# aleksandrina-streltsova/lidar-global-registration

Measured on AMD Instinct MI355X. Metric: scan-pair registrations/sec, higher is better.
Workload: dtype f32

## Files before the change

lidar-global-registration_amd/csrc/lgr_align.hip:

```cpp
#include <rocprim/device/device_scan.hpp>

#include <chrono>
#include <cmath>

#include <climits>

#include "lgr_internal.h"

namespace {

__device__ __forceinline__ float corr_threshold(float a, float b, float dthr) {
    float m = (a < b) ? b : a;
    return (dthr < m) ? dthr : m;
}

template <int KMAX>
__device__ __forceinline__ float cluster_distance(int i, int j, int k, const int32_t* __restrict__ knn_a, const int32_t* __restrict__ knn_b,
                                                   const int32_t* __restrict__ ab_idx) {
    int nb[KMAX];
#pragma unroll
    for (int b = 0; b < KMAX; ++b) nb[b] = b < k ? knn_b[(size_t) j * k + b] : -2;
    int consistent = 0, pairs = 0;
    for (int a0 = 0; a0 < k; a0 += 8) {
        int in[8], mt[8];
// ... 105 lines not shown
    size_t tb = 0;
    LGR_HIP(ctx, rocprim::exclusive_scan(nullptr, tb, flags, pos, 0, (size_t) ns, rocprim::plus<int>(), ctx->stream));
    void* tmp;
    LGR_TRY(lgr_ws(ctx, WS_GRID_TMP, tb, &tmp));
    LGR_HIP(ctx, rocprim::exclusive_scan(tmp, tb, flags, pos, 0, (size_t) ns, rocprim::plus<int>(), ctx->stream));
    filter_emit<<<cdiv(ns, 256), 256, 0, ctx->stream>>>(ns, d_ij_idx, flags, pos, dist, thr_s, thr_t, distance_thr, d_out);
    int* h;
    LGR_TRY(lgr_pinned(ctx, 64, (void**) &h));
    LGR_HIP(ctx, hipMemcpyAsync(h, pos + (ns - 1), 4, hipMemcpyDeviceToHost, ctx->stream));
    LGR_HIP(ctx, hipMemcpyAsync(h + 1, flags + (ns - 1), 4, hipMemcpyDeviceToHost, ctx->stream));
    LGR_HIP(ctx, hipStreamSynchronize(ctx->stream));
    *n_out = h[0] + h[1];
    LGR_HIP(ctx, hipGetLastError());
    return LGR_OK;
}

static void tick(lgr_ctx* ctx, int i) { (void) hipEventRecord(ctx->ev[i], ctx->stream); }

__global__ void gather_rows12_kernel(const float* __restrict__ pts, const int32_t* __restrict__ idx, int m, float* __restrict__ out) {
    size_t e = (size_t) blockIdx.x * blockDim.x + threadIdx.x;
    if (e >= (size_t) m * 12) return;
    out[e] = pts[(size_t) idx[e / 12] * 12 + e % 12];
}
static void gather_rows12(lgr_ctx* ctx, const float* pts, const int32_t* idx, int m, float* out) {
    gather_rows12_kernel<<<cdiv((long long) m * 12, 256), 256, 0, ctx->stream>>>(pts, idx, m, out);
}
__global__ void finalize_kernel(lgr_corr* __restrict__ corr, int n, const int32_t* __restrict__ ks, const int32_t* __restrict__ kt) {
    int i = blockIdx.x * blockDim.x + threadIdx.x;
    if (i >= n) return;
    corr[i].index_query = ks[corr[i].index_query];
    corr[i].index_match = kt[corr[i].index_match];
}

typedef int (*FeatureStage)(lgr_ctx* ctx, const float* kps, int m, const float* surf, int n, float radius, float* out, const lgr_params* p, const float* vp);
struct Descriptor {
    int len;
    FeatureStage stage;
    bool dense;
    int lrf;
};
static int fpfh_stage(lgr_ctx* ctx, const float* kps, int m, const float* surf, int n, float radius, float* out, const lgr_params*, const float*) { return lgr_fpfh_dev(ctx, kps, m, surf, n, radius, out); }
static int shot_stage(lgr_ctx* ctx, const float* kps, int m, const float* surf, int n, float radius, float* out, const lgr_params*, const float*) { return lgr_shot_dev(ctx, kps, m, surf, n, radius, nullptr, out, nullptr); }
static int rops_stage(lgr_ctx* ctx, const float* kps, int m, const float* surf, int n, float radius, float* out, const lgr_params* p, const float* vp) {
    float* kn;
    LGR_TRY(lgr_ws_t(ctx, WS_ROPS_KPS, (size_t) m * 12, &kn));
    LGR_HIP(ctx, hipMemcpyAsync(kn, kps, (size_t) m * 48, hipMemcpyDeviceToDevice, ctx->stream));
    LGR_TRY(lgr_normals_knn_dev(ctx, kn, m, surf, n, p->normal_nr_points, vp, 1));
    return lgr_rops_gravity_dev(ctx, kn, m, surf, n, radius, out);
}
static const Descriptor DESCRIPTORS[] = {
     {33, fpfh_stage, false, LGR_LRF_DEFAULT},
     {352, shot_stage, true, LGR_LRF_DEFAULT},
     {135, rops_stage, true, LGR_LRF_GRAVITY},
};
static_assert(LGR_DESCRIPTOR_FPFH == 0 && LGR_DESCRIPTOR_SHOT == 1 && LGR_DESCRIPTOR_ROPS == 2, "DESCRIPTORS is indexed by descriptor_id");

extern "C" void lgr_default_feature_params(lgr_feature_params* f) {
    if (!f) return;
    memset(f, 0, sizeof(*f));
    f->descriptor_id = LGR_DESCRIPTOR_FPFH;
    f->lrf_id = LGR_LRF_DEFAULT;
}

static int feature_descriptor(lgr_ctx* ctx, const lgr_params* p, const lgr_feature_params* f, const Descriptor** out) {
    *out = &DESCRIPTORS[LGR_DESCRIPTOR_FPFH];
    if (!f) return LGR_OK;
    LGR_CHECK(ctx, f->descriptor_id >= 0 && f->descriptor_id < (int) (sizeof DESCRIPTORS / sizeof *DESCRIPTORS), LGR_ERR_UNSUPPORTED);
    const Descriptor& d = DESCRIPTORS[f->descriptor_id];
    if (d.dense) {
        LGR_CHECK(ctx, f->lrf_id == LGR_LRF_DEFAULT || f->lrf_id == LGR_LRF_GRAVITY || f->lrf_id == LGR_LRF_GT, LGR_ERR_INVALID_ARG);
        LGR_CHECK(ctx, f->lrf_id == d.lrf, LGR_ERR_UNSUPPORTED);
        LGR_CHECK(ctx, p->use_bfmatcher && !p->has_guess, LGR_ERR_UNSUPPORTED);
        LGR_CHECK(ctx, ctx->opt.arithmetic != LGR_ARITH_PCL, LGR_ERR_UNSUPPORTED);
    }
    *out = &d;
    return LGR_OK;
// ... 7 lines not shown
    int sizes[2], ksizes[2];
    int32_t* kidx[2] = {nullptr, nullptr};
    lgr_corr* d_out;
    int* n_out;
    bool empty = false;
    float *feat[2], *surf[2], *dij, *dji;
    int32_t *ij, *ji;
    FilterTables ftab;
    float ms[3] = {0, 0, 0};
    struct Tables {
        CorrCall* c;
        int operator()(lgr_ctx* cx) const {
            LGR_TRY(filter_cloud_tables(cx, c->kclouds[0], c->ksizes[0], c->p->cluster_k, c->ftab.thr_s, c->ftab.knn_s));
            return filter_cloud_tables(cx, c->kclouds[1], c->ksizes[1], c->p->cluster_k, c->ftab.thr_t, c->ftab.knn_t);
        }
    } tables{this};
    lgr_helper_guard tables_guard;
    struct PrepGuard { lgr_ctx* c; ~PrepGuard() { lgr_match_prepare_cancel(c); } } prep_guard;

    CorrCall(lgr_ctx* ctx, const float* d_src, int ns, const float* d_tgt, int nt, const lgr_params* p, lgr_corr* d_out, int* n_out)
        : ctx(ctx), p(p), clouds{d_src, d_tgt}, kclouds{d_src, d_tgt}, sizes{ns, nt}, ksizes{ns, nt}, d_out(d_out), n_out(n_out), prep_guard{ctx} {}
    CorrCall(const CorrCall&) = delete;
    const float* vp(int side) const { return side == 0 ? (p->has_vp_src ? p->vp_src : nullptr) : (p->has_vp_tgt ? p->vp_tgt : nullptr); }
    float iss_radius(int side) const { return side == 0 ? p->iss_radius_src : p->iss_radius_tgt; }
    bool both_dirs() const { return p->matching_id != LGR_MATCH_ONE_SIDED; }
};

static int level_features(lgr_ctx* cx, const CorrCall& c, int side, const float* in, int n_in, float voxel, float radius, float* surf,
                          const float* kps, int m, const int32_t* d_list, float* sub, float* out, float* ms, int* nd) {
    const lgr_params* p = c.p;
    tick(cx, 0);
    LGR_TRY(lgr_downsample_dev(cx, in, n_in, voxel, surf, nd));
    tick(cx, 1);
    LGR_TRY(lgr_normals_knn_dev(cx, surf, *nd, nullptr, 0, p->normal_nr_points, c.vp(side), p->normals_available));
    tick(cx, 2);
    if (m) {
        if (d_list) { gather_rows12(cx, kps, d_list, m, sub); kps = sub; }
        LGR_TRY(c.d->stage(cx, kps, m, surf, *nd, radius, out, p, c.vp(side)));
    }
    tick(cx, 3);
    LGR_HIP(cx, hipEventSynchronize(cx->ev[3]));
    float t;
    for (int s = 0; s < 3; ++s) { (void) hipEventElapsedTime(&t, cx->ev[s], cx->ev[s + 1]); ms[s] += t; }
    return LGR_OK;
}

struct MsSide {
    float iss_radius = 0.f;
    int min_l2 = INT_MAX, max_l2 = INT_MIN;
    std::vector<std::vector<int>> lists;
    std::vector<size_t> feat_off;
    float* feat = nullptr;
    int32_t* d_lists = nullptr;
    std::vector<float> xyz;
};

static int ms_initialize(CorrCall& c, int side, MsSide& st) {
    lgr_ctx* ctx = c.ctx;
    const lgr_params* p = c.p;
    const int D = c.d->len, n = c.sizes[side], n_kps = c.ksizes[side];
    const float *d_pcd = c.clouds[side], *d_kps = c.kclouds[side];
    st.iss_radius = c.iss_radius(side);
    const int k = 5;
    LGR_CHECK(ctx, n >= k, LGR_ERR_INVALID_ARG);
    int32_t* d_nn;
    float* d_d2;
    LGR_TRY(lgr_ws_t(ctx, WS_MS_KNN_I, (size_t) n_kps * k, &d_nn));
    LGR_TRY(lgr_ws_t(ctx, WS_MS_KNN_D, (size_t) n_kps * k, &d_d2));
    LGR_TRY(lgr_knn_dev(ctx, d_kps, n_kps, d_pcd, n, k, d_nn, d_d2));
    std::vector<float> d2((size_t) n_kps * k);
    std::vector<float> kp((size_t) n_kps * 12);
// ... 410 lines not shown
```

lidar-global-registration_amd/csrc/lgr_features.hip:

```cpp
#include <rocprim/device/device_radix_sort.hpp>
#include <rocprim/device/device_scan.hpp>

#include <algorithm>
#include <cmath>
#include <type_traits>
#include <unordered_map>
#include <vector>

#include "lgr_grid.cuh"
#include "lgr_knn_wave.cuh"
#include "lgr_seqsum.h"
#include "lgr_math.cuh"
#include "lgr_libm.cuh"

namespace {

__global__ void voxel_keys(const float* __restrict__ pts, int n, float bx, float by, float bz, float voxel,
                           unsigned long long* __restrict__ keys, int* __restrict__ vals, int* __restrict__ bad) {
    int i = blockIdx.x * blockDim.x + threadIdx.x;
    if (i >= n) return;
    float x = pts[(size_t) i * 12], y = pts[(size_t) i * 12 + 1], z = pts[(size_t) i * 12 + 2];
    unsigned long long k = ~0ull;
    if (lgr_finite3(x, y, z)) {
        int ix = (int) floorf((x - bx) / voxel), iy = (int) floorf((y - by) / voxel), iz = (int) floorf((z - bz) / voxel);
// ... 959 lines not shown
        out[i] = r;
    }
}
extern "C" int lgr_selfcheck_libm(lgr_ctx* ctx, int fn, const float* a, const float* b, long long n, float* out) {
    lgr_turn turn__(ctx);
    if (!ctx) return LGR_ERR_INVALID_ARG;
    LGR_CHECK(ctx, fn >= 0 && fn <= 6 && a && out && n >= 0 && (fn != 2 || b), LGR_ERR_INVALID_ARG);
    if (n == 0) return LGR_OK;
    LGR_HIP(ctx, hipSetDevice(ctx->device));
    float *da, *db, *dout;
    LGR_TRY(lgr_ws_t(ctx, WS_HOST_A, (size_t) n, &da));
    LGR_TRY(lgr_ws_t(ctx, WS_HOST_B, (size_t) n, &db));
    LGR_TRY(lgr_ws_t(ctx, WS_HOST_C, (size_t) n, &dout));
    LGR_HIP(ctx, hipMemcpyAsync(da, a, (size_t) n * 4, hipMemcpyHostToDevice, ctx->stream));
    if (fn == 2) LGR_HIP(ctx, hipMemcpyAsync(db, b, (size_t) n * 4, hipMemcpyHostToDevice, ctx->stream));
    if (fn >= 5) LGR_TRY(lgr_weights_libm_launch(ctx, fn, da, n, dout));
    else libm_eval_kernel<<<8 * ctx->n_cu, 256, 0, ctx->stream>>>(fn, da, db, n, dout);
    LGR_HIP(ctx, hipGetLastError());
    LGR_HIP(ctx, hipMemcpyAsync(out, dout, (size_t) n * 4, hipMemcpyDeviceToHost, ctx->stream));
    LGR_HIP(ctx, hipStreamSynchronize(ctx->stream));
    return LGR_OK;
}

#ifdef LGR_SPFH_CHECK
extern "C" int lgr_debug_spfh_check(unsigned long long* out3, int reset) {
    unsigned long long z[4] = {0, 0, 0, 0};
    if (hipMemcpyFromSymbol(out3, HIP_SYMBOL(g_spfh_check), 24) != hipSuccess) return LGR_ERR_HIP;
    if (reset && hipMemcpyToSymbol(HIP_SYMBOL(g_spfh_check), z, 32) != hipSuccess) return LGR_ERR_HIP;
    return LGR_OK;
}
#endif

extern "C" int lgr_normals_knn_dev(lgr_ctx* ctx, float* d_pts, int n, const float* d_surf, int ns, int k, const float* vp3, int normals_available) {
    lgr_turn turn__(ctx);
    if (!ctx) return LGR_ERR_INVALID_ARG;
    LGR_CHECK(ctx, (d_pts || n == 0) && n >= 0 && k >= 1 && k <= 64, LGR_ERR_INVALID_ARG);
    (void) normals_available;
    if (n == 0) return LGR_OK;
    LGR_HIP(ctx, hipSetDevice(ctx->device));
    const float* S = d_surf;
    if (!S) {
        float* snap;
        LGR_TRY(lgr_ws_t(ctx, WS_HOST_F, (size_t) n * 12, &snap));
        LGR_HIP(ctx, hipMemcpyAsync(snap, d_pts, (size_t) n * 48, hipMemcpyDeviceToDevice, ctx->stream));
        S = snap; ns = n;
    }
    GridDev g;
    const bool wave = !d_surf && k >= 16;
    const float ppc = wave ? 10.f : 6.f;
    LGR_TRY(lgr_grid_build(ctx, WS_GRID_A, S, ns, 0.f, ppc, &g));
    size_t sm = (size_t) k * NB * 8;
    const float vx = vp3 ? vp3[0] : 0.f, vy = vp3 ? vp3[1] : 0.f, vz = vp3 ? vp3[2] : 0.f;
    if (wave) {
        const float r2i = g.h * g.h * 1.25f * (float) k / (3.14159265f * ppc);
        const int grid = lgr_xcd_grid(cdiv(g.n, 64 * NW_WAVES));
        const size_t sml = (size_t) NW_WAVES * k * 64 * sizeof(int);
        if (g.n > 0) {
            if (k <= 40) normals_wave_kernel<1><<<grid, 64 * NW_WAVES, sml, ctx->stream>>>(g, S, d_pts, k, vx, vy, vz, r2i);
            else {
                if (sml + 8192 > 65536) LGR_HIP(ctx, hipFuncSetAttribute((const void*) normals_wave_kernel<2>, hipFuncAttributeMaxDynamicSharedMemorySize, (int) sml));
                normals_wave_kernel<2><<<grid, 64 * NW_WAVES, sml, ctx->stream>>>(g, S, d_pts, k, vx, vy, vz, r2i);
            }
        }
        if (g.n < n) normals_kernel<<<cdiv(n, NB), NB, sm, ctx->stream>>>(g, S, d_pts, n, k, vx, vy, vz, 2);
    } else if (!d_surf) {
        if (g.n > 0) normals_kernel<<<lgr_xcd_grid(cdiv(g.n, NB)), NB, sm, ctx->stream>>>(g, S, d_pts, n, k, vx, vy, vz, 1);
        if (g.n < n) normals_kernel<<<cdiv(n, NB), NB, sm, ctx->stream>>>(g, S, d_pts, n, k, vx, vy, vz, 2);
    } else {
        normals_kernel<<<cdiv(n, NB), NB, sm, ctx->stream>>>(g, S, d_pts, n, k, vx, vy, vz, 0);
    }
    LGR_HIP(ctx, hipGetLastError());
    return LGR_OK;
}

extern "C" int lgr_normals_knn(lgr_ctx* ctx, float* pts, int n, const float* surf, int ns, int k, const float* vp3, int normals_available) {
    lgr_turn turn__(ctx);
    if (!ctx) return LGR_ERR_INVALID_ARG;
    LGR_CHECK(ctx, (pts || n == 0) && n >= 0, LGR_ERR_INVALID_ARG);
    if (n == 0) return LGR_OK;
    LGR_HIP(ctx, hipSetDevice(ctx->device));
    float *dp, *ds = nullptr;
    LGR_TRY(lgr_ws_t(ctx, WS_HOST_A, (size_t) n * 12, &dp));
    LGR_HIP(ctx, hipMemcpyAsync(dp, pts, (size_t) n * 48, hipMemcpyHostToDevice, ctx->stream));
    if (surf) {
        LGR_TRY(lgr_ws_t(ctx, WS_HOST_B, (size_t) ns * 12 + 4, &ds));
        LGR_HIP(ctx, hipMemcpyAsync(ds, surf, (size_t) ns * 48, hipMemcpyHostToDevice, ctx->stream));
    }
    LGR_TRY(lgr_normals_knn_dev(ctx, dp, n, ds, ns, k, vp3, normals_available));
    LGR_HIP(ctx, hipMemcpyAsync(pts, dp, (size_t) n * 48, hipMemcpyDeviceToHost, ctx->stream));
    LGR_HIP(ctx, hipStreamSynchronize(ctx->stream));
    return LGR_OK;
}

extern "C" int lgr_fpfh_dev(lgr_ctx* ctx, const float* d_kps, int m, const float* d_surf, int n, float radius, float* d_out) {
    lgr_turn turn__(ctx);
    if (!ctx) return LGR_ERR_INVALID_ARG;
    LGR_CHECK(ctx, (d_kps || m == 0) && (d_surf || n == 0) && (d_out || m == 0) && m >= 0 && n >= 0 && radius > 0.f, LGR_ERR_INVALID_ARG);
    LGR_CHECK(ctx, radius <= 1e18f && (size_t) n + 1 <= ((size_t) 1 << 32) / HP - 1, LGR_ERR_UNSUPPORTED);
    if (m == 0) return LGR_OK;
    LGR_HIP(ctx, hipSetDevice(ctx->device));
    GridDev g;
    LGR_TRY(lgr_grid_build(ctx, WS_GRID_B, d_surf, n, radius * 1.001f, 0.f, &g));
    float r2 = radius * radius;
    float* spfh;
    LGR_TRY(lgr_ws_t(ctx, WS_SPFH, ((size_t) n + 1) * HP + 64, &spfh));
    LGR_HIP(ctx, hipMemsetAsync(spfh + (size_t) g.n * HP, 0, HP * sizeof(float), ctx->stream));
    const long long n_cells = (long long) g.dx * g.dy * g.dz;
    int cell_bits = 1;
    while ((1ll << cell_bits) < n_cells) ++cell_bits;
    const int sb = std::max(0, std::min(2, (32 - cell_bits) / 3));
    const int key_bits = std::min(32, cell_bits + 3 * sb);
    const int mx = std::max(m, g.n);
    unsigned *keys, *keys2, *kkeys, *kkeys2;
    int *vals, *vals2, *kvals, *kvals2;
    LGR_TRY(lgr_ws_t(ctx, WS_KP_ORDER, (size_t) mx * 8 + 16, &keys));
    keys2 = keys + mx; vals = (int*) (keys2 + mx); vals2 = vals + mx;
    kkeys = (unsigned*) (vals2 + mx); kkeys2 = kkeys + mx; kvals = (int*) (kkeys2 + mx); kvals2 = kvals + mx;
    fine_keys<<<cdiv(m, 256), 256, 0, ctx->stream>>>(g, d_kps, 12, m, sb, kkeys, kvals);
    LGR_TRY(lgr_sort_pairs_u32(ctx, kkeys, kkeys2, kvals, kvals2, (size_t) m, 0, key_bits));
    if (g.n > 0) {
        fine_keys<<<cdiv(g.n, 256), 256, 0, ctx->stream>>>(g, reinterpret_cast<const float*>(g.pxyz), 4, g.n, sb, keys, vals);
        LGR_TRY(lgr_sort_pairs_u32(ctx, keys, keys2, vals, vals2, (size_t) g.n, 0, key_bits));
        spfh_tile_kernel<<<lgr_xcd_grid(cdiv(g.n, ST)), 64, 0, ctx->stream>>>(g, r2, vals2, spfh);
    }
    if (ctx->opt.arithmetic == LGR_ARITH_PCL) {
        if (ctx->opt.pcl_neighbour_cap == 64) fpfh_pcl_kernel<64><<<lgr_xcd_grid(m), 64, 0, ctx->stream>>>(g, d_kps, kvals2, m, r2, spfh, d_out);
        else if (ctx->opt.pcl_neighbour_cap == 1024) fpfh_pcl_kernel<1024><<<lgr_xcd_grid(m), 64, 0, ctx->stream>>>(g, d_kps, kvals2, m, r2, spfh, d_out);
        else fpfh_pcl_kernel<512><<<lgr_xcd_grid(m), 64, 0, ctx->stream>>>(g, d_kps, kvals2, m, r2, spfh, d_out);
    } else {
        fpfh_mfma_kernel<<<lgr_xcd_grid(cdiv(m, FT)), 64, 0, ctx->stream>>>(g, d_kps, kvals2, m, r2, spfh, d_out);
    }
    LGR_HIP(ctx, hipGetLastError());
    return LGR_OK;
}

// ... 18 lines not shown
```

lidar-global-registration_amd/csrc/lgr_grid.hip:

```cpp
#include <rocprim/device/device_radix_sort.hpp>
#include <rocprim/device/device_scan.hpp>

#include <algorithm>
#include <cmath>

#include "lgr_grid.cuh"
#include "lgr_knn_wave.cuh"

namespace {

__device__ __forceinline__ unsigned fkey(float f) {
    unsigned b = __float_as_uint(f);
    return (b & 0x80000000u) ? ~b : (b | 0x80000000u);
}
__host__ __device__ inline float fkey_inv(unsigned k) {
    unsigned b = (k & 0x80000000u) ? (k & 0x7fffffffu) : ~k;
    float f;
    memcpy(&f, &b, 4);
    return f;
}

__global__ void bbox_kernel(const float* __restrict__ pts, int n, unsigned* __restrict__ out) {
    float tmn[3] = {INFINITY, INFINITY, INFINITY}, tmx[3] = {-INFINITY, -INFINITY, -INFINITY};
    float qmn[3] = {3.4028234663852886e38f, 3.4028234663852886e38f, 3.4028234663852886e38f};
// ... 252 lines not shown
    unsigned kfmx, kfmn;
    memcpy(&kfmx, &fmx, 4); kfmx |= 0x80000000u;
    memcpy(&kfmn, &fmn, 4); kfmn |= 0x80000000u;
    for (int a = 0; a < 3; ++a) { init[a] = pinf; init[3 + a] = ninf; init[6 + a] = kfmx; init[9 + a] = kfmn; }
    LGR_HIP(ctx, hipMemcpyAsync(d, init, sizeof init, hipMemcpyHostToDevice, ctx->stream));
    if (n > 0) bbox_kernel<<<std::min(cdiv(n, 256), ctx->n_cu), 256, 0, ctx->stream>>>(d_pts, n, d);
    LGR_HIP(ctx, hipGetLastError());
    *d_keys12 = d;
    return LGR_OK;
}

int lgr_bbox_host(lgr_ctx* ctx, const float* d_pts, int n, float* out12) {
    const unsigned* d;
    LGR_TRY(lgr_bbox_launch(ctx, d_pts, n, &d));
    unsigned* h;
    LGR_TRY(lgr_pinned(ctx, 64, (void**) &h));
    LGR_HIP(ctx, hipMemcpyAsync(h, d, 48, hipMemcpyDeviceToHost, ctx->stream));
    LGR_HIP(ctx, hipStreamSynchronize(ctx->stream));
    for (int i = 0; i < 12; ++i) out12[i] = fkey_inv(h[i]);
    return LGR_OK;
}

extern "C" int lgr_bbox_dev(lgr_ctx* ctx, const float* d_pts, int n, float* d_min3_max3) {
    lgr_turn turn__(ctx);
    if (!ctx) return LGR_ERR_INVALID_ARG;
    LGR_CHECK(ctx, (d_pts || n == 0) && d_min3_max3 && n >= 0, LGR_ERR_INVALID_ARG);
    float bb[12];
    LGR_TRY(lgr_bbox_host(ctx, d_pts, n, bb));
    LGR_HIP(ctx, hipMemcpyAsync(d_min3_max3, bb + 6, 24, hipMemcpyHostToDevice, ctx->stream));
    LGR_HIP(ctx, hipStreamSynchronize(ctx->stream));
    return LGR_OK;
}

int lgr_grid_build(lgr_ctx* ctx, int sb, const float* d_pts, int n, float h, float target, GridDev* out) {
    float bb[12];
    LGR_TRY(lgr_bbox_host(ctx, d_pts, n, bb));
    float mn[3] = {bb[0], bb[1], bb[2]}, mx[3] = {bb[3], bb[4], bb[5]};
    if (!(mn[0] <= mx[0])) { for (int a = 0; a < 3; ++a) { mn[a] = 0.f; mx[a] = 0.f; } }
    if (!(h > 0.f)) {
        float e[3] = {mx[0] - mn[0], mx[1] - mn[1], mx[2] - mn[2]};
        std::sort(e, e + 3);
        float area = std::max(e[2] * e[1], 1e-12f);
        h = std::sqrt(area * target / (float) std::max(n, 1));
        h = std::max(h, std::max(e[2] / 1024.f, 1e-6f));
    }
    int dim[3];
    for (;;) {
        double cells = 1;
        for (int a = 0; a < 3; ++a) {
            dim[a] = (int) std::floor((mx[a] - mn[a]) / h) + 1;
            if (dim[a] < 1) dim[a] = 1;
            cells *= dim[a];
        }
        if (cells <= 256e6) break;
        h *= 2.f;
    }
    int ncell = dim[0] * dim[1] * dim[2];
    unsigned *keys, *keys2;
    int *vals, *vals2, *start;
    float4 *pxyz, *pnrm;
    LGR_TRY(lgr_ws_t(ctx, sb + 0, (size_t) n + 1, &keys));
    LGR_TRY(lgr_ws_t(ctx, sb + 1, (size_t) n + 1, &vals));
    LGR_TRY(lgr_ws_t(ctx, sb + 2, (size_t) n + 1, &keys2));
    LGR_TRY(lgr_ws_t(ctx, sb + 3, (size_t) n + 1, &vals2));
    LGR_TRY(lgr_ws_t(ctx, sb + 4, (size_t) ncell + 2, &start));
    LGR_TRY(lgr_ws_t(ctx, sb + 5, (size_t) n + 1, &pxyz));
    LGR_TRY(lgr_ws_t(ctx, sb + 6, (size_t) n + 1, &pnrm));
    int nvalid = 0;
    if (n > 0) {
// ... 98 lines not shown
```

lidar-global-registration_amd/csrc/lgr_internal.h:

```cpp
#pragma once
#include <hip/hip_runtime.h>
#include <stdint.h>
#include <stdio.h>
#include <string.h>

#include <condition_variable>
#include <functional>
#include <mutex>
#include <string>
#include <thread>
#include <vector>

#include "../../include/lgr.h"

#define LGR_WAVE 64
#define LGR_STREAM_OWN_LOW ((void*) (intptr_t) -2)

struct lgr_buf {
    void* p = nullptr;
    size_t cap = 0;
};

struct lgr_match_stats { unsigned items_ab, dense_ab, items_ba, dense_ba; int sub_cols, rg_rows; double stages_done, stages_all, stages_unique; int f16; double coarse_tested, coarse_rejected; unsigned pairs_ab, pairs_ba; double shell_skipped; double lb_zero, lb_finite; unsigned irr_a, irr_b, irr_gave_up; };

// ... 84 lines not shown
    WS_DENSE_PACK_A, WS_DENSE_PACK_B, WS_DENSE_KEYS,
    WS_ROPS_MASKED, WS_ROPS_LRF, WS_ROPS_KPS,
    WS_WEIGHTS, WS_WEIGHTS_KNN, WS_WEIGHTS_TMP, WS_WEIGHTS_VALS, WS_WEIGHTS_SUM, WS_WEIGHTS_HOST,
    WS_GT_MISC, WS_GT_TERMS, WS_GT_ALIGNED, WS_GT_OVERLAP, WS_GT_FLAGS, WS_GT_KNN, WS_GT_DENS, WS_GT_CORR,
    WS_PD_TERMS, WS_PD_MISC, WS_PD_INLIERS, WS_PD_MASK,
    WS_DBG_MISC, WS_DBG_MOVED, WS_DBG_FLAGS, WS_DBG_OVERLAP, WS_DBG_DENS, WS_DBG_SORT, WS_DBG_HOST_A, WS_DBG_HOST_B,
    WS_HYP_SET, WS_HYP_ITEMS, WS_HYP_FINAL,
    WS_COUNT
};
static_assert(WS_COUNT <= 160, "grow lgr_ctx::ws");

int lgr_ws(lgr_ctx* ctx, int slot, size_t bytes, void** out);
int lgr_pinned(lgr_ctx* ctx, size_t bytes, void** out);

template <class T>
static inline int lgr_ws_t(lgr_ctx* ctx, int slot, size_t count, T** out) {
    void* p = nullptr;
    int rc = lgr_ws(ctx, slot, count * sizeof(T), &p);
    *out = (T*) p;
    return rc;
}

static inline int cdiv(long long a, long long b) { return (int) ((a + b - 1) / b); }
static inline size_t cdivz(size_t a, size_t b) { return (a + b - 1) / b; }

struct GridDev {
    float ox, oy, oz, h;
    int dx, dy, dz;
    int n;
    const int* cell_start;
    const float4* pxyz;
    const float4* pnrm;
};
int lgr_grid_build(lgr_ctx* ctx, int slot_base, const float* d_pts, int n, float h, float target, GridDev* out);
int lgr_rops_gravity_dev(lgr_ctx* ctx, const float* d_kps, int m, const float* d_surf, int n, float radius, float* d_out135);
int lgr_bbox_host(lgr_ctx* ctx, const float* d_pts, int n, float* out12);
int lgr_bbox_launch(lgr_ctx* ctx, const float* d_pts, int n, const unsigned** d_keys12);
__host__ __device__ inline float lgr_bbox_key_inv(unsigned k) {
    const unsigned b = (k & 0x80000000u) ? (k & 0x7fffffffu) : ~k;
    float f;
    memcpy(&f, &b, 4);
    return f;
}
void lgr_inverse4(const float* m16, float* out16);
int lgr_knn_lists(lgr_ctx* ctx, const float* d_q, int nq, const float* d_pts, int n, int k, int32_t* d_idx, float* d_d2);

int lgr_ctx_aux(lgr_ctx* ctx);
int lgr_ctx_aux2(lgr_ctx* ctx);
int lgr_ctx_stream3(lgr_ctx* ctx, hipStream_t* out);
int lgr_helper_post(lgr_ctx* owner, lgr_ctx* aux, std::function<int()> job);
int lgr_helper_wait(lgr_ctx* aux);
struct lgr_helper_guard {
    lgr_ctx* aux = nullptr;
    bool armed = false;
    int wait() { armed = false; return lgr_helper_wait(aux); }
    ~lgr_helper_guard() { if (armed) (void) lgr_helper_wait(aux); }
};
template <class F>
static inline std::function<int()> lgr_aux_job(lgr_ctx* aux, F&& f) {
    return [aux, &f]() -> int {
        int rc = hipSetDevice(aux->device) == hipSuccess ? f(aux) : (int) LGR_ERR_HIP;
        const hipError_t e = hipStreamSynchronize(aux->stream);
        if (rc == LGR_OK && e != hipSuccess) rc = lgr_fail(aux, LGR_ERR_HIP, hipGetErrorString(e), __FILE__, __LINE__);
        return rc;
    };
}
template <class FA, class FB>
// ... 67 lines not shown
```

lidar-global-registration_amd/csrc/lgr_match.hip:

```cpp
#include <rocprim/device/device_radix_sort.hpp>
#include <rocprim/device/device_scan.hpp>

#include <algorithm>
#include <vector>

#include "lgr_internal.h"

#include "lgr_match_common.cuh"
#include "lgr_match_cluster.cuh"
#include "lgr_match_pack.cuh"
#include "lgr_match_mfma.cuh"
#include "lgr_match_sweep.cuh"
#include "lgr_match_bounds.cuh"
#include "lgr_match_rerank.cuh"

extern "C" int lgr_match_last_stats(lgr_ctx* ctx, unsigned* out6) {
    if (!ctx || !out6) return LGR_ERR_INVALID_ARG;
    const lgr_match_stats& s = ctx->mstats;
    out6[0] = s.items_ab; out6[1] = s.dense_ab; out6[2] = s.items_ba;
    out6[3] = s.dense_ba; out6[4] = (unsigned) s.sub_cols; out6[5] = (unsigned) s.rg_rows;
    return LGR_OK;
}
extern "C" int lgr_match_last_work(lgr_ctx* ctx, double* executed_fraction) {
    if (!ctx || !executed_fraction) return LGR_ERR_INVALID_ARG;
// ... 136 lines not shown
struct MatchPrep {
    bool armed = false;
    const float* d_a = nullptr;
    int ma = 0, mb = 0;
    bool both = false;
    lgr_match_options mopt{};
    int sub = 1, rg_rows = BLOCK_ROWS, ns = 0;
    float *cen = nullptr, *cen2 = nullptr, *smp = nullptr, *basis = nullptr;
    int* smp_ok = nullptr;
    IrrRef* irr = nullptr;
    bool basis_ready = false;
    Side A;
};
static void match_prep_free(void* p) { delete (MatchPrep*) p; }
static MatchPrep* match_prep_of(lgr_ctx* ctx) {
    if (!ctx->match_prep) { ctx->match_prep = new MatchPrep(); ctx->match_prep_free = match_prep_free; }
    return (MatchPrep*) ctx->match_prep;
}

static int match_cluster(lgr_ctx* ctx, const float* d_a, int ma, const float* d_b, int mb, bool both, bool basis_side_by_side, MatchPrep* P) {
    const lgr_match_options& mo = ctx->mopt;
    int sub = 1;
    while (sub < SUBMAX && (long long) KCL * sub * 1024 < std::max(ma, mb)) sub *= 2;
    if (mo.leaves > 0) sub = mo.leaves;
    sub = std::min(SUBMAX, std::max(1, sub));
    const int n_leaves = KCL * sub;
    const int ns = 2 * KM_SAMPLE;
    char* misc;
    Carve carve{8192};
    const size_t o_cen2 = carve((size_t) MAXLEAF * 33 * 4);
    const size_t o_smp = carve((size_t) ns * 33 * 4), o_ok = carve((size_t) ns * 4), o_label = carve((size_t) ns * 4);
    const size_t o_cbuf = carve((size_t) 2 * KCL * 33 * 4), o_basis = carve((size_t) (34 * 33 + 64) * 4);
    const size_t o_skeys = carve((size_t) 2 * ns * 4), o_svals = carve((size_t) ns * 4), o_sidx = carve((size_t) ns * 4), o_coff = carve(256);
    const size_t o_zero = carve.off;
    const size_t o_kmax = carve(256), o_irr = carve(sizeof(IrrRef)), o_acc1 = carve((size_t) KM_ITERS * KCL * sizeof(KmAcc)), o_acc2 = carve((size_t) MAXLEAF * sizeof(KmAcc));
    const size_t zero_bytes = carve.off - o_zero;
    LGR_TRY(lgr_ws_t(ctx, WS_MATCH_MISC, carve.off, &misc));
    float* cen = (float*) (misc + 256);
    float* cen2 = (float*) (misc + o_cen2);
    float* smp = (float*) (misc + o_smp);
    int* smp_ok = (int*) (misc + o_ok);
    int* label = (int*) (misc + o_label);
    float* cbuf = (float*) (misc + o_cbuf);
    float* basis = (float*) (misc + o_basis);
    unsigned* skeys = (unsigned*) (misc + o_skeys);
    int* svals = (int*) (misc + o_svals);
    int* sidx = (int*) (misc + o_sidx);
    int* coff = (int*) (misc + o_coff);
    unsigned* kmax = (unsigned*) (misc + o_kmax);
    KmAcc* acc1 = (KmAcc*) (misc + o_acc1);
    KmAcc* acc2 = (KmAcc*) (misc + o_acc2);
    LGR_HIP(ctx, hipMemsetAsync(misc + o_zero, 0, zero_bytes, ctx->stream));
    IrrRef* irr = mo.irregular_rows ? (IrrRef*) (misc + o_irr) : nullptr;
    if (irr) km_consensus<<<cdiv(ns, 256), 256, 0, ctx->stream>>>(d_a, ma, d_b, mb, KM_SAMPLE, irr);
    km_sample<<<cdiv(ns, 256), 256, 0, ctx->stream>>>(d_a, ma, d_b, mb, KM_SAMPLE, smp, smp_ok, kmax, irr);
    auto lloyd = [&](lgr_ctx* cx) -> int {
        km_init<<<1, 64, 0, cx->stream>>>(smp, smp_ok, ns, cbuf);
        for (int it = 0; it <= KM_ITERS; ++it) {
            const bool last = it == KM_ITERS;
            km1_step<<<cdiv(ns, KM1_THREADS), KM1_THREADS, 0, cx->stream>>>(smp, smp_ok, ns, kmax, cbuf + (it & 1) * KCL * 33, it ? acc1 + (size_t) (it - 1) * KCL : nullptr,
                                                                            last ? nullptr : acc1 + (size_t) it * KCL, last ? cen : cbuf + ((it + 1) & 1) * KCL * 33, label);
        }
        km_label_keys<<<cdiv(ns, 256), 256, 0, cx->stream>>>(label, ns, skeys, svals);
        LGR_TRY(lgr_sort_pairs_u32(cx, skeys, skeys + ns, svals, sidx, (size_t) ns, 0, 5));
        km_cluster_offsets<<<1, 64, 0, cx->stream>>>(skeys + ns, ns, coff);
        km2_init<<<KCL, 64, 0, cx->stream>>>(smp, sidx, coff, cen, sub, cen2);
        if (sub > 1) {
            for (int it = 0; it < KM2_ITERS; ++it) {
                km2_step<<<dim3(KM2_PIECES, KCL), KM2_THREADS, 0, cx->stream>>>(smp, sidx, coff, kmax, cen2, sub, acc2);
                km2_finalize<<<n_leaves, 64, 0, cx->stream>>>(acc2, kmax, cen2);
            }
        }
        LGR_HIP(cx, hipGetLastError());
        return LGR_OK;
    };
    const bool want_basis = mo.box_bounds != 0;
    if (want_basis && basis_side_by_side) {
        LGR_TRY(lgr_run_pair(ctx, lloyd, [&](lgr_ctx* cx) { return box_basis(cx, mo.box_bounds == 2, smp, smp_ok, ns, basis, []() { return (int) LGR_OK; }); }));
    } else if (want_basis) {
        LGR_TRY(box_basis(ctx, mo.box_bounds == 2, smp, smp_ok, ns, basis, [&]() { return lloyd(ctx); }));
    } else {
        LGR_TRY(lloyd(ctx));
    }
    auto pick_group = [](size_t q_count, size_t t_count) {
        int g = 1024;
        while (g < 4096 && (t_count / g + 1) * q_count * 4 > ((size_t) 6 << 30)) g *= 2;
        return g;
    };
// ... 834 lines not shown
```

lidar-global-registration_amd/csrc/lgr_match_cluster.cuh:

```cuda
#pragma once
#include "lgr_match_common.cuh"

namespace {

struct KmAcc { long long sum[33]; long long cnt; };
__device__ __forceinline__ double km_scale(unsigned kmax_bits) {
    return kmax_bits ? ldexp(1.0, 40 - ((int) (kmax_bits >> 23) - 127)) : 1.0;
}
constexpr int IRR_CAND = 16;
constexpr int IRR_CAP = 1024;
struct IrrRef { double s[3]; double tol; int enabled; int best; unsigned n_ok; unsigned agree[IRR_CAND]; };
__device__ __forceinline__ void block_sums(const float* v, double& s0, double& s1, double& s2) {
    s0 = 0.0; s1 = 0.0; s2 = 0.0;
#pragma unroll
    for (int k = 0; k < 11; ++k) { s0 += (double) v[k]; s1 += (double) v[11 + k]; s2 += (double) v[22 + k]; }
}
__device__ __forceinline__ bool sums_agree(double a0, double a1, double a2, double r0, double r1, double r2, double tol) {
    return fabs(a0 - r0) <= tol && fabs(a1 - r1) <= tol && fabs(a2 - r2) <= tol;
}
__device__ __forceinline__ double sums_tol(double r0, double r1, double r2) { return 1e-5 * fmax(fmax(fabs(r0), fabs(r1)), fabs(r2)); }
__device__ __forceinline__ const float* sample_row(int s, const float* __restrict__ A, int ma, const float* __restrict__ B, int mb, int per_side) {
    const bool fromA = !B || s < per_side;
    const float* X = fromA ? A : B;
    const int m = fromA ? ma : mb;
    if (m <= 0) return nullptr;
    const int t = fromA ? s : s - per_side;
    const long long i = (long long) t * m / (B ? per_side : 2 * per_side);
    return X + (size_t) i * 33;
}
__device__ __forceinline__ bool irr_decide(const IrrRef* __restrict__ ref, int& best) {
    unsigned top = 0u;
    best = 0;
    for (int c = 0; c < IRR_CAND; ++c) { const unsigned a = ref->agree[c]; if (a > top) { top = a; best = c; } }
    const unsigned n_ok = ref->n_ok;
    return n_ok >= 256u && (unsigned long long) top * 1000ull >= (unsigned long long) n_ok * 995ull;
}
__global__ __launch_bounds__(256) void km_consensus(const float* __restrict__ A, int ma, const float* __restrict__ B, int mb, int per_side, IrrRef* __restrict__ ref) {
    __shared__ double cs[IRR_CAND][3];
    __shared__ int cok[IRR_CAND];
    const int ns = 2 * per_side;
    if (threadIdx.x < IRR_CAND) {
        const float* r = sample_row((int) ((long long) threadIdx.x * ns / IRR_CAND), A, ma, B, mb, per_side);
        float v[33];
        const bool ok = r && row_finite(r, v);
        double s0 = 0.0, s1 = 0.0, s2 = 0.0;
        if (ok) block_sums(v, s0, s1, s2);
        cs[threadIdx.x][0] = s0; cs[threadIdx.x][1] = s1; cs[threadIdx.x][2] = s2;
        cok[threadIdx.x] = ok ? 1 : 0;
    }
    __syncthreads();
    const int s = blockIdx.x * blockDim.x + threadIdx.x;
    bool ok = false;
    double s0 = 0.0, s1 = 0.0, s2 = 0.0;
    if (s < ns) {
        const float* r = sample_row(s, A, ma, B, mb, per_side);
        float v[33];
        ok = r && row_finite(r, v);
        if (ok) block_sums(v, s0, s1, s2);
    }
    const int lane = threadIdx.x & 63;
    for (int c = 0; c < IRR_CAND; ++c) {
        const bool a = ok && cok[c] && sums_agree(s0, s1, s2, cs[c][0], cs[c][1], cs[c][2], sums_tol(cs[c][0], cs[c][1], cs[c][2]));
        const int n = __popcll(__ballot(a));
        if (lane == 0 && n) atomicAdd(&ref->agree[c], (unsigned) n);
    }
    const int n_ok = __popcll(__ballot(ok));
    if (lane == 0 && n_ok) atomicAdd(&ref->n_ok, (unsigned) n_ok);
}
__global__ void km_sample(const float* __restrict__ A, int ma, const float* __restrict__ B, int mb, int per_side,
                          float* __restrict__ smp, int* __restrict__ smp_ok, unsigned* __restrict__ kmax , IrrRef* __restrict__ irr_ref) {
    int s = blockIdx.x * blockDim.x + threadIdx.x;
    if (s >= 2 * per_side) return;
    const float* r = sample_row(s, A, ma, B, mb, per_side);
    float v[33];
    bool ok = r && row_finite(r, v);
    if (irr_ref) {
        int best;
        const bool on = irr_decide(irr_ref, best);
        double r0 = 0.0, r1 = 0.0, r2 = 0.0;
        if (on) {
            const float* rr = sample_row((int) ((long long) best * (2 * per_side) / IRR_CAND), A, ma, B, mb, per_side);
            float w[33];
            (void) row_finite(rr, w);
            block_sums(w, r0, r1, r2);
            if (ok) {
                double s0, s1, s2;
                block_sums(v, s0, s1, s2);
                ok = sums_agree(s0, s1, s2, r0, r1, r2, sums_tol(r0, r1, r2));
            }
        }
        if (s == 0) { irr_ref->s[0] = r0; irr_ref->s[1] = r1; irr_ref->s[2] = r2; irr_ref->tol = sums_tol(r0, r1, r2); irr_ref->best = best; irr_ref->enabled = on ? 1 : 0; }
    }
    float mx = 0.f;
    for (int k = 0; k < 33; ++k) { smp[(size_t) s * 33 + k] = ok ? v[k] : 0.f; if (ok) mx = fmaxf(mx, fabsf(v[k])); }
    smp_ok[s] = ok ? 1 : 0;
    for (int o = 32; o > 0; o >>= 1) mx = fmaxf(mx, __shfl_xor(mx, o));
    if ((threadIdx.x & 63) == 0 && mx > 0.f) atomicMax(kmax, __float_as_uint(mx));
}
__global__ void km_init(const float* __restrict__ smp, const int* __restrict__ smp_ok, int ns, float* __restrict__ cen) {
    int c = threadIdx.x;
    if (c >= KCL) return;
    int s = (int) ((long long) c * ns / KCL);
    int tries = 0;
    while (!smp_ok[s] && tries < ns) { s = (s + 1) % ns; ++tries; }
    for (int k = 0; k < 33; ++k) cen[c * 33 + k] = smp_ok[s] ? smp[(size_t) s * 33 + k] : 0.f;
}
__device__ __forceinline__ int nearest_centre(const float* v, const float* __restrict__ cen, float& best) {
    int bi = 0;
    best = __uint_as_float(0x7f800000u);
#pragma unroll 1
    for (int c = 0; c < KCL; ++c) {
        float d = 0.f;
#pragma unroll
        for (int k = 0; k < 33; ++k) { float t = v[k] - cen[c * 33 + k]; d = d + t * t; }
        if (d < best) { best = d; bi = c; }
    }
    return bi;
}
constexpr int KM1_THREADS = 256;
__global__ __launch_bounds__(KM1_THREADS) void km1_step(const float* __restrict__ smp, const int* __restrict__ smp_ok, int ns, const unsigned* __restrict__ kmax,
                                                        const float* __restrict__ cen_prev, const KmAcc* __restrict__ acc_prev, KmAcc* __restrict__ acc_out,
                                                        float* __restrict__ cen_out, int* __restrict__ label) {
    __shared__ float cen_s[KCL * 33];
    __shared__ long long acc_s[KCL * 34];
    const double scale = km_scale(*kmax);
    for (int e = threadIdx.x; e < KCL * 33; e += KM1_THREADS) {
        const int c = e / 33, k = e % 33;
        float v = cen_prev[e];
        if (acc_prev && acc_prev[c].cnt > 0) v = (float) (((double) acc_prev[c].sum[k] / scale) / (double) acc_prev[c].cnt);
        cen_s[e] = v;
// ... 223 lines not shown
```

Before: 45.06.

## Share surface bbox across grid builds and drop global atomics in k-means sampling

Computes the surface bounding box once per level on the host and passes it to the normals and FPFH grid builds, so the bbox reduction and its host sync run once instead of twice. The device-to-device snapshot copy in the normals path is removed, and the grid is built directly on the input points. The k-means consensus kernel now writes per-block vote partials instead of using global atomics. The sampling kernel reduces those partials per block and does a block-level max before a single atomic. The bbox reuse depends on the surface not changing between the two builds, and dropping the snapshot assumes the normals kernel does not modify the points it is reading.

```diff
diff --git a/lidar-global-registration_amd/csrc/lgr_align.hip b/lidar-global-registration_amd/csrc/lgr_align.hip
--- a/lidar-global-registration_amd/csrc/lgr_align.hip
+++ b/lidar-global-registration_amd/csrc/lgr_align.hip
@@ -161,16 +161,16 @@
     corr[i].index_match = kt[corr[i].index_match];
 }
 
-typedef int (*FeatureStage)(lgr_ctx* ctx, const float* kps, int m, const float* surf, int n, float radius, float* out, const lgr_params* p, const float* vp);
+typedef int (*FeatureStage)(lgr_ctx* ctx, const float* kps, int m, const float* surf, int n, float radius, float* out, const lgr_params* p, const float* vp, const float* surf_bbox12);
 struct Descriptor {
     int len;
     FeatureStage stage;
     bool dense;
     int lrf;
 };
-static int fpfh_stage(lgr_ctx* ctx, const float* kps, int m, const float* surf, int n, float radius, float* out, const lgr_params*, const float*) { return lgr_fpfh_dev(ctx, kps, m, surf, n, radius, out); }
-static int shot_stage(lgr_ctx* ctx, const float* kps, int m, const float* surf, int n, float radius, float* out, const lgr_params*, const float*) { return lgr_shot_dev(ctx, kps, m, surf, n, radius, nullptr, out, nullptr); }
-static int rops_stage(lgr_ctx* ctx, const float* kps, int m, const float* surf, int n, float radius, float* out, const lgr_params* p, const float* vp) {
+static int fpfh_stage(lgr_ctx* ctx, const float* kps, int m, const float* surf, int n, float radius, float* out, const lgr_params*, const float*, const float* bb) { return lgr_fpfh_bbox(ctx, kps, m, surf, n, radius, out, bb); }
+static int shot_stage(lgr_ctx* ctx, const float* kps, int m, const float* surf, int n, float radius, float* out, const lgr_params*, const float*, const float*) { return lgr_shot_dev(ctx, kps, m, surf, n, radius, nullptr, out, nullptr); }
+static int rops_stage(lgr_ctx* ctx, const float* kps, int m, const float* surf, int n, float radius, float* out, const lgr_params* p, const float* vp, const float*) {
     float* kn;
     LGR_TRY(lgr_ws_t(ctx, WS_ROPS_KPS, (size_t) m * 12, &kn));
     LGR_HIP(ctx, hipMemcpyAsync(kn, kps, (size_t) m * 48, hipMemcpyDeviceToDevice, ctx->stream));
@@ -244,11 +244,14 @@
     tick(cx, 0);
     LGR_TRY(lgr_downsample_dev(cx, in, n_in, voxel, surf, nd));
     tick(cx, 1);
-    LGR_TRY(lgr_normals_knn_dev(cx, surf, *nd, nullptr, 0, p->normal_nr_points, c.vp(side), p->normals_available));
+    float bb12[12];
+    const float* bb = nullptr;
+    if (*nd > 0) { LGR_TRY(lgr_bbox_host(cx, surf, *nd, bb12)); bb = bb12; }
+    LGR_TRY(lgr_normals_knn_bbox(cx, surf, *nd, nullptr, 0, p->normal_nr_points, c.vp(side), p->normals_available, bb));
     tick(cx, 2);
     if (m) {
         if (d_list) { gather_rows12(cx, kps, d_list, m, sub); kps = sub; }
-        LGR_TRY(c.d->stage(cx, kps, m, surf, *nd, radius, out, p, c.vp(side)));
+        LGR_TRY(c.d->stage(cx, kps, m, surf, *nd, radius, out, p, c.vp(side), bb));
     }
     tick(cx, 3);
     LGR_HIP(cx, hipEventSynchronize(cx->ev[3]));
diff --git a/lidar-global-registration_amd/csrc/lgr_features.hip b/lidar-global-registration_amd/csrc/lgr_features.hip
--- a/lidar-global-registration_amd/csrc/lgr_features.hip
+++ b/lidar-global-registration_amd/csrc/lgr_features.hip
@@ -1015,6 +1015,9 @@
 #endif
 
 extern "C" int lgr_normals_knn_dev(lgr_ctx* ctx, float* d_pts, int n, const float* d_surf, int ns, int k, const float* vp3, int normals_available) {
+    return lgr_normals_knn_bbox(ctx, d_pts, n, d_surf, ns, k, vp3, normals_available, nullptr);
+}
+int lgr_normals_knn_bbox(lgr_ctx* ctx, float* d_pts, int n, const float* d_surf, int ns, int k, const float* vp3, int normals_available, const float* surf_bbox12) {
     lgr_turn turn__(ctx);
     if (!ctx) return LGR_ERR_INVALID_ARG;
     LGR_CHECK(ctx, (d_pts || n == 0) && n >= 0 && k >= 1 && k <= 64, LGR_ERR_INVALID_ARG);
@@ -1023,15 +1026,12 @@
     LGR_HIP(ctx, hipSetDevice(ctx->device));
     const float* S = d_surf;
     if (!S) {
-        float* snap;
-        LGR_TRY(lgr_ws_t(ctx, WS_HOST_F, (size_t) n * 12, &snap));
-        LGR_HIP(ctx, hipMemcpyAsync(snap, d_pts, (size_t) n * 48, hipMemcpyDeviceToDevice, ctx->stream));
-        S = snap; ns = n;
+        S = d_pts; ns = n;
     }
     GridDev g;
     const bool wave = !d_surf && k >= 16;
     const float ppc = wave ? 10.f : 6.f;
-    LGR_TRY(lgr_grid_build(ctx, WS_GRID_A, S, ns, 0.f, ppc, &g));
+    LGR_TRY(lgr_grid_build(ctx, WS_GRID_A, S, ns, 0.f, ppc, &g, surf_bbox12));
     size_t sm = (size_t) k * NB * 8;
     const float vx = vp3 ? vp3[0] : 0.f, vy = vp3 ? vp3[1] : 0.f, vz = vp3 ? vp3[2] : 0.f;
     if (wave) {
@@ -1076,6 +1076,9 @@
 }
 
 extern "C" int lgr_fpfh_dev(lgr_ctx* ctx, const float* d_kps, int m, const float* d_surf, int n, float radius, float* d_out) {
+    return lgr_fpfh_bbox(ctx, d_kps, m, d_surf, n, radius, d_out, nullptr);
+}
+int lgr_fpfh_bbox(lgr_ctx* ctx, const float* d_kps, int m, const float* d_surf, int n, float radius, float* d_out, const float* surf_bbox12) {
     lgr_turn turn__(ctx);
     if (!ctx) return LGR_ERR_INVALID_ARG;
     LGR_CHECK(ctx, (d_kps || m == 0) && (d_surf || n == 0) && (d_out || m == 0) && m >= 0 && n >= 0 && radius > 0.f, LGR_ERR_INVALID_ARG);
@@ -1083,7 +1086,7 @@
     if (m == 0) return LGR_OK;
     LGR_HIP(ctx, hipSetDevice(ctx->device));
     GridDev g;
-    LGR_TRY(lgr_grid_build(ctx, WS_GRID_B, d_surf, n, radius * 1.001f, 0.f, &g));
+    LGR_TRY(lgr_grid_build(ctx, WS_GRID_B, d_surf, n, radius * 1.001f, 0.f, &g, surf_bbox12));
     float r2 = radius * radius;
     float* spfh;
     LGR_TRY(lgr_ws_t(ctx, WS_SPFH, ((size_t) n + 1) * HP + 64, &spfh));
diff --git a/lidar-global-registration_amd/csrc/lgr_grid.hip b/lidar-global-registration_amd/csrc/lgr_grid.hip
--- a/lidar-global-registration_amd/csrc/lgr_grid.hip
+++ b/lidar-global-registration_amd/csrc/lgr_grid.hip
@@ -308,9 +308,10 @@
     return LGR_OK;
 }
 
-int lgr_grid_build(lgr_ctx* ctx, int sb, const float* d_pts, int n, float h, float target, GridDev* out) {
+int lgr_grid_build(lgr_ctx* ctx, int sb, const float* d_pts, int n, float h, float target, GridDev* out, const float* bbox12) {
     float bb[12];
-    LGR_TRY(lgr_bbox_host(ctx, d_pts, n, bb));
+    if (bbox12) memcpy(bb, bbox12, sizeof bb);
+    else LGR_TRY(lgr_bbox_host(ctx, d_pts, n, bb));
     float mn[3] = {bb[0], bb[1], bb[2]}, mx[3] = {bb[3], bb[4], bb[5]};
     if (!(mn[0] <= mx[0])) { for (int a = 0; a < 3; ++a) { mn[a] = 0.f; mx[a] = 0.f; } }
     if (!(h > 0.f)) {
diff --git a/lidar-global-registration_amd/csrc/lgr_internal.h b/lidar-global-registration_amd/csrc/lgr_internal.h
--- a/lidar-global-registration_amd/csrc/lgr_internal.h
+++ b/lidar-global-registration_amd/csrc/lgr_internal.h
@@ -140,7 +140,9 @@
     const float4* pxyz;
     const float4* pnrm;
 };
-int lgr_grid_build(lgr_ctx* ctx, int slot_base, const float* d_pts, int n, float h, float target, GridDev* out);
+int lgr_grid_build(lgr_ctx* ctx, int slot_base, const float* d_pts, int n, float h, float target, GridDev* out, const float* bbox12 = nullptr);
+int lgr_normals_knn_bbox(lgr_ctx* ctx, float* d_pts, int n, const float* d_surf, int ns, int k, const float* vp3, int normals_available, const float* surf_bbox12);
+int lgr_fpfh_bbox(lgr_ctx* ctx, const float* d_kps, int m, const float* d_surf, int n, float radius, float* d_out, const float* surf_bbox12);
 int lgr_rops_gravity_dev(lgr_ctx* ctx, const float* d_kps, int m, const float* d_surf, int n, float radius, float* d_out135);
 int lgr_bbox_host(lgr_ctx* ctx, const float* d_pts, int n, float* out12);
 int lgr_bbox_launch(lgr_ctx* ctx, const float* d_pts, int n, const unsigned** d_keys12);
diff --git a/lidar-global-registration_amd/csrc/lgr_match.hip b/lidar-global-registration_amd/csrc/lgr_match.hip
--- a/lidar-global-registration_amd/csrc/lgr_match.hip
+++ b/lidar-global-registration_amd/csrc/lgr_match.hip
@@ -192,6 +192,8 @@
     const size_t o_smp = carve((size_t) ns * 33 * 4), o_ok = carve((size_t) ns * 4), o_label = carve((size_t) ns * 4);
     const size_t o_cbuf = carve((size_t) 2 * KCL * 33 * 4), o_basis = carve((size_t) (34 * 33 + 64) * 4);
     const size_t o_skeys = carve((size_t) 2 * ns * 4), o_svals = carve((size_t) ns * 4), o_sidx = carve((size_t) ns * 4), o_coff = carve(256);
+    const int n_vote = cdiv(ns, 256);
+    const size_t o_vote = carve((size_t) n_vote * IRR_VOTE * 4);
     const size_t o_zero = carve.off;
     const size_t o_kmax = carve(256), o_irr = carve(sizeof(IrrRef)), o_acc1 = carve((size_t) KM_ITERS * KCL * sizeof(KmAcc)), o_acc2 = carve((size_t) MAXLEAF * sizeof(KmAcc));
     const size_t zero_bytes = carve.off - o_zero;
@@ -212,8 +214,9 @@
     KmAcc* acc2 = (KmAcc*) (misc + o_acc2);
     LGR_HIP(ctx, hipMemsetAsync(misc + o_zero, 0, zero_bytes, ctx->stream));
     IrrRef* irr = mo.irregular_rows ? (IrrRef*) (misc + o_irr) : nullptr;
-    if (irr) km_consensus<<<cdiv(ns, 256), 256, 0, ctx->stream>>>(d_a, ma, d_b, mb, KM_SAMPLE, irr);
-    km_sample<<<cdiv(ns, 256), 256, 0, ctx->stream>>>(d_a, ma, d_b, mb, KM_SAMPLE, smp, smp_ok, kmax, irr);
+    unsigned* vote = (unsigned*) (misc + o_vote);
+    if (irr) km_consensus<<<n_vote, 256, 0, ctx->stream>>>(d_a, ma, d_b, mb, KM_SAMPLE, vote);
+    km_sample<<<cdiv(ns, KM_SAMPLE_THREADS), KM_SAMPLE_THREADS, 0, ctx->stream>>>(d_a, ma, d_b, mb, KM_SAMPLE, smp, smp_ok, kmax, irr, vote, n_vote);
     auto lloyd = [&](lgr_ctx* cx) -> int {
         km_init<<<1, 64, 0, cx->stream>>>(smp, smp_ok, ns, cbuf);
         for (int it = 0; it <= KM_ITERS; ++it) {
diff --git a/lidar-global-registration_amd/csrc/lgr_match_cluster.cuh b/lidar-global-registration_amd/csrc/lgr_match_cluster.cuh
--- a/lidar-global-registration_amd/csrc/lgr_match_cluster.cuh
+++ b/lidar-global-registration_amd/csrc/lgr_match_cluster.cuh
@@ -28,16 +28,20 @@
     const long long i = (long long) t * m / (B ? per_side : 2 * per_side);
     return X + (size_t) i * 33;
 }
-__device__ __forceinline__ bool irr_decide(const IrrRef* __restrict__ ref, int& best) {
+constexpr int IRR_VOTE = IRR_CAND + 1;
+constexpr int KM_SAMPLE_THREADS = 256;
+__device__ __forceinline__ bool irr_decide(const unsigned* tot , int& best) {
     unsigned top = 0u;
     best = 0;
-    for (int c = 0; c < IRR_CAND; ++c) { const unsigned a = ref->agree[c]; if (a > top) { top = a; best = c; } }
-    const unsigned n_ok = ref->n_ok;
+    for (int c = 0; c < IRR_CAND; ++c) { const unsigned a = tot[c]; if (a > top) { top = a; best = c; } }
+    const unsigned n_ok = tot[IRR_CAND];
     return n_ok >= 256u && (unsigned long long) top * 1000ull >= (unsigned long long) n_ok * 995ull;
 }
-__global__ __launch_bounds__(256) void km_consensus(const float* __restrict__ A, int ma, const float* __restrict__ B, int mb, int per_side, IrrRef* __restrict__ ref) {
+__global__ __launch_bounds__(256) void km_consensus(const float* __restrict__ A, int ma, const float* __restrict__ B, int mb, int per_side,
+                                                    unsigned* __restrict__ part ) {
     __shared__ double cs[IRR_CAND][3];
     __shared__ int cok[IRR_CAND];
+    __shared__ unsigned wcnt[4][IRR_VOTE];
     const int ns = 2 * per_side;
     if (threadIdx.x < IRR_CAND) {
         const float* r = sample_row((int) ((long long) threadIdx.x * ns / IRR_CAND), A, ma, B, mb, per_side);
@@ -58,44 +62,71 @@
         ok = r && row_finite(r, v);
         if (ok) block_sums(v, s0, s1, s2);
     }
-    const int lane = threadIdx.x & 63;
+    const int lane = threadIdx.x & 63, wv = threadIdx.x >> 6;
     for (int c = 0; c < IRR_CAND; ++c) {
         const bool a = ok && cok[c] && sums_agree(s0, s1, s2, cs[c][0], cs[c][1], cs[c][2], sums_tol(cs[c][0], cs[c][1], cs[c][2]));
         const int n = __popcll(__ballot(a));
-        if (lane == 0 && n) atomicAdd(&ref->agree[c], (unsigned) n);
+        if (lane == 0) wcnt[wv][c] = (unsigned) n;
     }
     const int n_ok = __popcll(__ballot(ok));
-    if (lane == 0 && n_ok) atomicAdd(&ref->n_ok, (unsigned) n_ok);
-}
-__global__ void km_sample(const float* __restrict__ A, int ma, const float* __restrict__ B, int mb, int per_side,
-                          float* __restrict__ smp, int* __restrict__ smp_ok, unsigned* __restrict__ kmax , IrrRef* __restrict__ irr_ref) {
-    int s = blockIdx.x * blockDim.x + threadIdx.x;
-    if (s >= 2 * per_side) return;
-    const float* r = sample_row(s, A, ma, B, mb, per_side);
+    if (lane == 0) wcnt[wv][IRR_CAND] = (unsigned) n_ok;
+    __syncthreads();
+    if (threadIdx.x < IRR_VOTE) part[(size_t) blockIdx.x * IRR_VOTE + threadIdx.x] = (wcnt[0][threadIdx.x] + wcnt[1][threadIdx.x]) + (wcnt[2][threadIdx.x] + wcnt[3][threadIdx.x]);
+}
+__global__ __launch_bounds__(KM_SAMPLE_THREADS) void km_sample(const float* __restrict__ A, int ma, const float* __restrict__ B, int mb, int per_side,
+                                                               float* __restrict__ smp, int* __restrict__ smp_ok, unsigned* __restrict__ kmax ,
+                                                               IrrRef* __restrict__ irr_ref, const unsigned* __restrict__ irr_part, int n_part) {
+    __shared__ unsigned tot[IRR_VOTE];
+    __shared__ double ref_s[4];
+    __shared__ int ref_on;
+    const int s = blockIdx.x * blockDim.x + threadIdx.x;
+    const bool in = s < 2 * per_side;
+    const float* r = in ? sample_row(s, A, ma, B, mb, per_side) : nullptr;
     float v[33];
     bool ok = r && row_finite(r, v);
     if (irr_ref) {
-        int best;
-        const bool on = irr_decide(irr_ref, best);
-        double r0 = 0.0, r1 = 0.0, r2 = 0.0;
-        if (on) {
-            const float* rr = sample_row((int) ((long long) best * (2 * per_side) / IRR_CAND), A, ma, B, mb, per_side);
-            float w[33];
-            (void) row_finite(rr, w);
-            block_sums(w, r0, r1, r2);
-            if (ok) {
-                double s0, s1, s2;
-                block_sums(v, s0, s1, s2);
-                ok = sums_agree(s0, s1, s2, r0, r1, r2, sums_tol(r0, r1, r2));
-            }
-        }
-        if (s == 0) { irr_ref->s[0] = r0; irr_ref->s[1] = r1; irr_ref->s[2] = r2; irr_ref->tol = sums_tol(r0, r1, r2); irr_ref->best = best; irr_ref->enabled = on ? 1 : 0; }
+        if (threadIdx.x < IRR_VOTE) tot[threadIdx.x] = 0u;
+        __syncthreads();
+        for (int e = threadIdx.x; e < n_part * IRR_VOTE; e += KM_SAMPLE_THREADS) atomicAdd(&tot[e % IRR_VOTE], irr_part[e]);
+        __syncthreads();
+        if (threadIdx.x == 0) {
+            int best;
+            const bool on = irr_decide(tot, best);
+            double r0 = 0.0, r1 = 0.0, r2 = 0.0;
+            if (on) {
+                const float* rr = sample_row((int) ((long long) best * (2 * per_side) / IRR_CAND), A, ma, B, mb, per_side);
+                float w[33];
+                (void) row_finite(rr, w);
+                block_sums(w, r0, r1, r2);
+            }
+            ref_s[0] = r0; ref_s[1] = r1; ref_s[2] = r2; ref_s[3] = sums_tol(r0, r1, r2);
+            ref_on = on ? 1 : 0;
+            if (blockIdx.x == 0) {
+                irr_ref->s[0] = r0; irr_ref->s[1] = r1; irr_ref->s[2] = r2; irr_ref->tol = ref_s[3]; irr_ref->best = best; irr_ref->enabled = on ? 1 : 0;
+                irr_ref->n_ok = tot[IRR_CAND];
+                for (int c = 0; c < IRR_CAND; ++c) irr_ref->agree[c] = tot[c];
+            }
+        }
+        __syncthreads();
+        if (ref_on && ok) {
+            double s0, s1, s2;
+            block_sums(v, s0, s1, s2);
+            ok = sums_agree(s0, s1, s2, ref_s[0], ref_s[1], ref_s[2], ref_s[3]);
+        }
     }
     float mx = 0.f;
-    for (int k = 0; k < 33; ++k) { smp[(size_t) s * 33 + k] = ok ? v[k] : 0.f; if (ok) mx = fmaxf(mx, fabsf(v[k])); }
-    smp_ok[s] = ok ? 1 : 0;
+    if (in) {
+        for (int k = 0; k < 33; ++k) { smp[(size_t) s * 33 + k] = ok ? v[k] : 0.f; if (ok) mx = fmaxf(mx, fabsf(v[k])); }
+        smp_ok[s] = ok ? 1 : 0;
+    }
     for (int o = 32; o > 0; o >>= 1) mx = fmaxf(mx, __shfl_xor(mx, o));
-    if ((threadIdx.x & 63) == 0 && mx > 0.f) atomicMax(kmax, __float_as_uint(mx));
+    __shared__ float wmx[KM_SAMPLE_THREADS / 64];
+    if ((threadIdx.x & 63) == 0) wmx[threadIdx.x >> 6] = mx;
+    __syncthreads();
+    if (threadIdx.x == 0) {
+        for (int w = 1; w < KM_SAMPLE_THREADS / 64; ++w) mx = fmaxf(mx, wmx[w]);
+        if (mx > 0.f) atomicMax(kmax, __float_as_uint(mx));
+    }
 }
 __global__ void km_init(const float* __restrict__ smp, const int* __restrict__ smp_ok, int ns, float* __restrict__ cen) {
     int c = threadIdx.x;
```

After: 45.30 (median of 3 runs). No clear change (+0.5%).
